# yuxiaoxiangyong/Multilateral-Temporal-view-Pyramid-Transformer-for-Video-Inpainting-Detection

Measured on AMD Instinct MI355X. Metric: clips/sec fwd (B=8,T=5,224x224), higher is better.
Workload: dtype f32; 1 GPU; full Mumpy forward (3 temporal views, pyramid decoder), B=8 clips/GPU, T=5, 224x224, fp32, tubelets (5,4,1); global_batch=8, launch=hipGraph replay, fork/join over HIP streams (independent branches co-scheduled), parallelism=batch-sharded x1, one metric all-reduce

## Files before the change

### include/mumpy_hip.h

```cpp
#ifndef MUMPY_HIP_H
#define MUMPY_HIP_H

#include <stdint.h>

#ifdef __cplusplus
extern "C" {
#endif

#define MUMPY_ABI_VERSION 2

#define MUMPY_EINVAL   (-1)
#define MUMPY_EALIGN   (-2)
#define MUMPY_ENULL    (-3)
#define MUMPY_ERANGE   (-4)

#define MUMPY_ACT_NONE 0
#define MUMPY_ACT_GELU 1
#define MUMPY_MATH_BF16 0x100
#define MUMPY_MATH_BF16X3 0x200
#define MUMPY_MATH_BF16X2 0x400

int         mumpy_abi_version(void);
const char* mumpy_last_error(void);
int         mumpy_tuning_build(void);
// ... 3 lines not shown
int mumpy_linear_rd_fwd(const float* x, const float* W, const float* bias, const float* residual, float* y, int64_t M, int N, int K,
                        int act, void* stream);
int mumpy_window_attention_bg_fwd(const float* qkv, float* out, const float* bias, const float* mask_tab, const int32_t* mask_id,
                                  int n_mask, int B, int Hs, int W, int C, int shift, float scale, void* stream);

int mumpy_linear_ln_tiles(int64_t M, int N, int K);
int mumpy_linear_lnx_fwd(const float* x, const float* W, const float* bias, const float* residual, float* y, int64_t M, int N, int K,
                         int act, void* workspace, int64_t workspace_bytes, float* stats_out, const float* ln_stats, int ln_gn,
                         const float* ln_colsum, float ln_eps, void* stream);

int mumpy_deform_sample_kv_fwd(const float* x2, const float* pos, const float* Wkv, const float* bkv, float* kv, int B, int Hs2,
                               int W, int C, int nq, void* stream);

int mumpy_deform_out_combine_fwd(const float* o, const float* Wout, const float* bout, const float* x1, float* out, int B, int H,
                                 int W, int C, void* stream);

int mumpy_avgpool2_pad_nhwc_fwd(const float* x, float* out, int B, int H, int W, int C, int Cpad, int nchw_in, void* stream);

int mumpy_copy_rows_fwd(const float* src, int64_t src_stride, float* dst, int64_t dst_stride, int64_t rows, int cols, void* stream);

int mumpy_merge_views_fwd(const float* v1, const float* v2, const float* v3, float* out, int B, int T, int n, int C1, int C2,
                          int C3, int t1, int t2, int t3, void* stream);

int mumpy_trunk_head_fwd(const float* g, const float* f, const float* gcn, const float* freq, float* z, int B, int h, int w, int C,
                         void* stream);

int mumpy_layernorm_fwd(const float* x, const float* gamma, const float* beta, float* y,
                        int64_t rows, int C, float eps, void* stream);

int mumpy_layernorm_bf16_fwd(const float* x, const float* gamma, const float* beta, void* y,
// ... 194 lines not shown
```

### multilateral-temporal-view-pyramid-transformer-for-video-inpainting-detection_amd/csrc/abi.cpp

```cpp
#include <stdarg.h>
#include <stdio.h>
#include "common.h"

namespace mumpy {
static thread_local char g_err[512] = "";
void set_error(const char* fmt, ...) {
    va_list ap;
    va_start(ap, fmt);
    vsnprintf(g_err, sizeof(g_err), fmt, ap);
    va_end(ap);
}
#ifdef MUMPY_TUNING
#include <stdlib.h>
int tune_int(const char* name, int dflt) {
    const char* v = getenv(name);
    return v ? atoi(v) : dflt;
}
const char* tune_str(const char* name) { return getenv(name); }
#endif
}

extern "C" int mumpy_tuning_build(void) {
#ifdef MUMPY_TUNING
    return 1;
#else
    return 0;
#endif
}

extern "C" int mumpy_abi_version(void) { return MUMPY_ABI_VERSION; }
extern "C" const char* mumpy_last_error(void) { return mumpy::g_err; }
```

### multilateral-temporal-view-pyramid-transformer-for-video-inpainting-detection_amd/csrc/cva_fused.hip

```cpp
#include "common.h"
using namespace mumpy;

namespace {

constexpr int BK = 32, LDR = 36;

__device__ __forceinline__ void divmod49(unsigned m, unsigned& q, unsigned& r) {
    q = (unsigned)(((uint64_t)m * 2804876602ull) >> 37);
    r = m - 49u * q;
}

template <int C>
__global__ __launch_bounds__(256, 2) void deform_sample_kv_kernel(const float* __restrict__ x2, const float* __restrict__ pos,
                                                                  const float* __restrict__ Wkv, const float* __restrict__ bkv,
                                                                  float* __restrict__ kv, int Hs2, int W, int nWx, int nW2, int nq,
                                                                  int M, unsigned gn) {
    constexpr int BM = 64, BN = 192, TN = 3, N = 2 * C, K = C, CG = C / 3, NK = K / BK, CPG = CG / BK;
    constexpr int A_LD = BM / 32, B_LD = BN / 32;
    __shared__ __attribute__((aligned(16))) float lds[2][(BM + BN) * LDR];
    const int tid = threadIdx.x, lane = tid & 63, wave = tid >> 6;
    const int c = lane & 31, h = lane >> 5, wm = wave >> 1, wn = wave & 1;
    const unsigned nwg = gridDim.x, orig = blockIdx.x, xcd = orig & 7, q8 = nwg >> 3, r8 = nwg & 7;
    const unsigned wgid = (xcd < r8 ? xcd * (q8 + 1) : r8 * (q8 + 1) + (xcd - r8) * q8) + (orig >> 3);
    const unsigned tm = wgid / gn, tn = wgid - tm * gn;
// ... 5 lines not shown
    int aoff[A_LD][4];
    float aw[A_LD][4];
#pragma unroll
    for (int i = 0; i < A_LD; ++i) {
        int m = m0 + ld_row + 32 * i;
        if (m > M - 1) m = M - 1;
        unsigned b2, p;
        divmod49((unsigned)m, b2, p);
        const unsigned b = b2 / (unsigned)nW2, n = b2 - b * (unsigned)nW2;
        const unsigned wy = n / (unsigned)nWx, wx = n - wy * (unsigned)nWx;
        abase[i] = x2 + (((int64_t)b * Hs2 + wy * WS) * W + wx * WS) * C + 4 * ld_c4;
        apos[i] = pos + ((int64_t)(b2 % (unsigned)nq) * 3 * WT + p) * 2;
    }
    auto set_group = [&](int g) {
#pragma unroll
        for (int i = 0; i < A_LD; ++i) {
            const float gy = apos[i][g * WT * 2], gx = apos[i][g * WT * 2 + 1];
            const float iy = ((gy + 1.0f) * 0.5f) * 6.0f;
            const float ix = ((gx + 1.0f) * 0.5f) * 6.0f;
            const float y0f = floorf(iy), x0f = floorf(ix);
            const int y0 = (int)y0f, x0 = (int)x0f;
            const float wgt[4] = {(x0f + 1.0f - ix) * (y0f + 1.0f - iy), (ix - x0f) * (y0f + 1.0f - iy),
                                  (x0f + 1.0f - ix) * (iy - y0f), (ix - x0f) * (iy - y0f)};
#pragma unroll
            for (int e = 0; e < 4; ++e) {
                const int yy = y0 + (e >> 1), xx = x0 + (e & 1);
                const bool ok = (unsigned)yy < (unsigned)WS && (unsigned)xx < (unsigned)WS;
                aw[i][e] = ok ? wgt[e] : 0.f;
                aoff[i][e] = ok ? (yy * W + xx) * C : 0;
            }
        }
    };
    const float* brow[B_LD];
#pragma unroll
    for (int i = 0; i < B_LD; ++i) {
        int n = n0 + ld_row + 32 * i;
        if (n > N - 1) n = N - 1;
        brow[i] = Wkv + (int64_t)n * K + 4 * ld_c4;
    }
    f32x4 areg[A_LD], breg[B_LD];
    auto gload = [&](int kc) {
        const int k0 = kc * BK;
#pragma unroll
        for (int i = 0; i < A_LD; ++i) {
            const float* s = abase[i] + k0;
            f32x4 r = *reinterpret_cast<const f32x4*>(s + aoff[i][0]) * aw[i][0];
            r += *reinterpret_cast<const f32x4*>(s + aoff[i][1]) * aw[i][1];
            r += *reinterpret_cast<const f32x4*>(s + aoff[i][2]) * aw[i][2];
            r += *reinterpret_cast<const f32x4*>(s + aoff[i][3]) * aw[i][3];
            areg[i] = r;
        }
#pragma unroll
        for (int i = 0; i < B_LD; ++i) breg[i] = *reinterpret_cast<const f32x4*>(brow[i] + k0);
    };
    auto lstore = [&](int buf) {
#pragma unroll
        for (int i = 0; i < A_LD; ++i) *reinterpret_cast<f32x4*>(&lds[buf][(ld_row + 32 * i) * LDR + 4 * ld_c4]) = areg[i];
#pragma unroll
        for (int i = 0; i < B_LD; ++i) *reinterpret_cast<f32x4*>(&lds[buf][(BM + ld_row + 32 * i) * LDR + 4 * ld_c4]) = breg[i];
    };
    f32x16 acc[TN];
#pragma unroll
    for (int j = 0; j < TN; ++j)
#pragma unroll
        for (int r = 0; r < 16; ++r) acc[j][r] = 0.f;
// ... 109 lines not shown
    const unsigned b = bw / (unsigned)nWf, n = bw - b * (unsigned)nWf;
    const int wy = (int)(n / (unsigned)nWx), wx = (int)(n - (n / (unsigned)nWx) * (unsigned)nWx);
    const int64_t img = (int64_t)b * H * W;
    const int64_t win_base = (img + (int64_t)n * WT) * C;
#pragma unroll
    for (int r = 0; r < 16; ++r) {
        const int cc = c0 + wm * 32 + (r & 3) + 8 * (r >> 2) + 4 * h;
        if (cc >= C) continue;
        const int f = cc * WT + (int)pp;
        const int po = f / C, co = f - po * C;
        const int tok = window_token(wy, wx, po, H, W, 0);
        out[win_base + f] = x1[win_base + f] + x1[(img + tok) * C + co] + (acc[r] + bout[cc]);
    }
}

}

extern "C" int mumpy_deform_sample_kv_fwd(const float* x2, const float* pos, const float* Wkv, const float* bkv, float* kv, int B,
                                          int Hs2, int W, int C, int nq, void* stream) {
    MUMPY_REQUIRE(x2 && pos && Wkv && bkv && kv, MUMPY_ENULL, "deform_sample_kv: null pointer");
    MUMPY_REQUIRE(aligned16(x2) && aligned16(Wkv) && aligned16(kv), MUMPY_EALIGN, "deform_sample_kv: pointers must be 16-byte aligned");
    MUMPY_REQUIRE(B > 0 && Hs2 > 0 && W > 0 && Hs2 % WS == 0 && W % WS == 0 && nq > 0, MUMPY_EINVAL,
                  "deform_sample_kv: bad grid (%d,%d) / nq=%d", Hs2, W, nq);
    MUMPY_REQUIRE(C == 96 || C == 192 || C == 384 || C == 768, MUMPY_EINVAL,
                  "deform_sample_kv: C=%d is not one of the encoder widths 96/192/384/768", C);
    const int nWx = W / WS, nW2 = (Hs2 / WS) * nWx;
    const int64_t nwin = (int64_t)B * nW2, M = nwin * WT;
    MUMPY_REQUIRE(M < (1ll << 31) - 64, MUMPY_ERANGE, "deform_sample_kv: too many windows");
    const unsigned gn = (unsigned)((2 * C + 191) / 192);
    const int64_t grid = ((M + 63) / 64) * gn;
    MUMPY_REQUIRE(grid < (1ll << 31), MUMPY_ERANGE, "deform_sample_kv: too many tiles");
#define MUMPY_SKV(C_)                                                                                                     \
    hipLaunchKernelGGL(deform_sample_kv_kernel<C_>, dim3((unsigned)grid), dim3(256), 0, as_stream(stream), x2, pos, Wkv, bkv, \
                       kv, Hs2, W, nWx, nW2, nq, (int)M, gn)
    switch (C) {
        case 96: MUMPY_SKV(96); break;
        case 192: MUMPY_SKV(192); break;
        case 384: MUMPY_SKV(384); break;
        default: MUMPY_SKV(768); break;
    }
#undef MUMPY_SKV
    MUMPY_CHECK_LAUNCH("deform_sample_kv");
    return 0;
}

extern "C" int mumpy_deform_out_combine_fwd(const float* o, const float* Wout, const float* bout, const float* x1, float* out, int B,
                                            int H, int W, int C, void* stream) {
    MUMPY_REQUIRE(o && Wout && bout && x1 && out, MUMPY_ENULL, "deform_out_combine: null pointer");
    MUMPY_REQUIRE(x1 != out, MUMPY_EINVAL, "deform_out_combine: out must not alias x1");
    MUMPY_REQUIRE(aligned16(o) && aligned16(Wout), MUMPY_EALIGN, "deform_out_combine: pointers must be 16-byte aligned");
    MUMPY_REQUIRE(B > 0 && H > 0 && W > 0 && H % WS == 0 && W % WS == 0, MUMPY_EINVAL, "deform_out_combine: bad grid (%d,%d)", H, W);
    MUMPY_REQUIRE(C == 96 || C == 192 || C == 384 || C == 768, MUMPY_EINVAL,
                  "deform_out_combine: C=%d is not one of the encoder widths 96/192/384/768", C);
    const int nWx = W / WS, nWf = (H / WS) * nWx;
    const int64_t MO = (int64_t)B * nWf * WT;
    MUMPY_REQUIRE(MO * 49 < (1ll << 31) && MO < (1ll << 31) - 64, MUMPY_ERANGE, "deform_out_combine: too many windows");
    const unsigned gn = (unsigned)((C + 63) / 64);
    const int64_t grid = ((MO + 63) / 64) * gn;
#define MUMPY_OC(C_)                                                                                                      \
    hipLaunchKernelGGL(deform_out_combine_kernel<C_>, dim3((unsigned)grid), dim3(256), 0, as_stream(stream), o, Wout, bout, x1, \
                       out, H, W, nWx, nWf, (int)MO, gn)
    switch (C) {
        case 96: MUMPY_OC(96); break;
        case 192: MUMPY_OC(192); break;
        case 384: MUMPY_OC(384); break;
        default: MUMPY_OC(768); break;
    }
#undef MUMPY_OC
    MUMPY_CHECK_LAUNCH("deform_out_combine");
    return 0;
}
```

### multilateral-temporal-view-pyramid-transformer-for-video-inpainting-detection_amd/csrc/deform.hip

```cpp
#include <stdlib.h>
#include "common.h"
using namespace mumpy;

namespace {

template <int Cg>
__global__ __launch_bounds__(256) void deform_offsets_kernel(const float* __restrict__ q, const float* __restrict__ dw_w,
                                                             const float* __restrict__ dw_b,
                                                             const float* __restrict__ ln_g,
                                                             const float* __restrict__ ln_b,
                                                             const float* __restrict__ pw_w, float* __restrict__ pos,
                                                             int H, int W, int C, int nWx, int nWf) {
    constexpr int CP = Cg + 4;
    __shared__ __attribute__((aligned(16))) float sm[WT * Cg + WT * CP + 25 * Cg + 4 * Cg];
    float* tile = sm;
    float* conv = sm + WT * Cg;
    float* wsm = conv + WT * CP;
    float* par = wsm + 25 * Cg;
    const int bw = blockIdx.x, g = blockIdx.y;
    const int b = bw / nWf, n = bw - b * nWf;
    const int wy = n / nWx, wx = n - wy * nWx;
    const int tid = threadIdx.x;
    const int64_t L = (int64_t)H * W;
    const float* qb = q + (int64_t)b * L * C + g * Cg;
// ... 73 lines not shown
        for (int ch = qd; ch < Cg; ch += 4) {
            const float a = gelu_erf((cv[ch] - mean) * rstd * par[ch] + par[Cg + ch]);
            oy = fmaf(a, par[2 * Cg + ch], oy);
            ox = fmaf(a, par[3 * Cg + ch], ox);
        }
        oy += __shfl_xor(oy, 1);
        oy += __shfl_xor(oy, 2);
        ox += __shfl_xor(ox, 1);
        ox += __shfl_xor(ox, 2);
        if (qd == 0) {
            const int py = p / WS, px = p - py * WS;
            const float ry = ((0.5f + (float)py) / 7.0f) * 2.0f - 1.0f;
            const float rx = ((0.5f + (float)px) / 7.0f) * 2.0f - 1.0f;
            const float rng = 1.0f / 7.0f;
            float* o = pos + (((int64_t)bw * 3 + g) * WT + p) * 2;
            o[0] = tanhf(oy) * rng * 2.0f + ry;
            o[1] = tanhf(ox) * rng * 2.0f + rx;
        }
    }
}

template <int C>
__global__ __launch_bounds__(256) void deform_sample_kernel(const float* __restrict__ x2, const float* __restrict__ pos,
                                                            float* __restrict__ out, int Hs2, int W, int nWx, int nW2,
                                                            int nq) {
    constexpr int C4N = C / 4, CG = C / 3;
    const int b2 = blockIdx.x;
    const int b = b2 / nW2, n = b2 - b * nW2;
    const int wy = n / nWx, wx = n - wy * nWx;
    const float* base = x2 + ((int64_t)b * Hs2 * W + (int64_t)wy * WS * W + wx * WS) * C;
// ... 98 lines not shown
        reinterpret_cast<f32x4*>(o)[i] = reinterpret_cast<const f32x4*>(a)[i] + reinterpret_cast<const f32x4*>(b)[i];
}

}

extern "C" int mumpy_deform_offsets_fwd(const float* q, const float* dw_w, const float* dw_b, const float* ln_g,
                                        const float* ln_b, const float* pw_w, float* pos, int B, int H, int W, int C,
                                        void* stream) {
    MUMPY_REQUIRE(q && dw_w && dw_b && ln_g && ln_b && pw_w && pos, MUMPY_ENULL, "deform_offsets: null pointer");
    MUMPY_REQUIRE(aligned16(q) && aligned16(dw_w), MUMPY_EALIGN, "deform_offsets: q and the depthwise weights must be 16-byte aligned");
    MUMPY_REQUIRE(B > 0 && H % WS == 0 && W % WS == 0 && H > 0 && W > 0, MUMPY_EINVAL, "deform_offsets: bad grid (%d,%d)", H, W);
    const int Cg = C / 3;
    MUMPY_REQUIRE(C % 3 == 0 && (Cg == 32 || Cg == 64 || Cg == 128 || Cg == 256), MUMPY_EINVAL,
                  "deform_offsets: group width C/3=%d must be 32, 64, 128 or 256", Cg);
    const int nWx = W / WS, nWf = (H / WS) * nWx;
#define MUMPY_OFFS(CG)                                                                                              \
    hipLaunchKernelGGL(deform_offsets_kernel<CG>, dim3(B * nWf, 3), dim3(256), 0, as_stream(stream), q, dw_w, dw_b, ln_g, \
                       ln_b, pw_w, pos, H, W, C, nWx, nWf)
    switch (Cg) {
        case 32: MUMPY_OFFS(32); break;
        case 64: MUMPY_OFFS(64); break;
        case 128: MUMPY_OFFS(128); break;
        default: MUMPY_OFFS(256); break;
    }
#undef MUMPY_OFFS
    MUMPY_CHECK_LAUNCH("deform_offsets");
    return 0;
}

extern "C" int mumpy_deform_sample_fwd(const float* x2, const float* pos, float* out, int B, int Hs2, int W, int C,
                                       int nq, void* stream) {
    MUMPY_REQUIRE(x2 && pos && out, MUMPY_ENULL, "deform_sample: null pointer");
    MUMPY_REQUIRE(aligned16(x2) && aligned16(out), MUMPY_EALIGN, "deform_sample: pointers must be 16-byte aligned");
// ... 51 lines not shown
```

### multilateral-temporal-view-pyramid-transformer-for-video-inpainting-detection_amd/csrc/window_attention.hip

```cpp
#include <stdlib.h>
#include <type_traits>
#include "common.h"
using namespace mumpy;

namespace {

struct SelfArgs {
    const float* qkv;
    float* out;
    const float* bias;
    const float* mask_tab;
    const int32_t* mask_id;
    int B, Hs, W, C, nH, shift, nWx, nW, n_mask, groups, stagger;
    int dbg;
    float scale;
    int64_t units;
};

struct CrossArgs {
    const float* q;
    const float* kv;
    const float* padmask;
    float* out;
    int B, H, W, C, nH, r, nWx, nWf, B1w;
// ... 464 lines not shown
#pragma unroll
        for (int it = 0; it < 2; ++it) {
            f32x16 s[2];
#pragma unroll
            for (int jt = 0; jt < 2; ++jt)
#pragma unroll
                for (int r = 0; r < 16; ++r) s[jt][r] = 0.f;
            qk_product(s, kf, qf[it]);
            bias_softmax<false>(s, [&](int jt, int g) {
                f32x4 bv = {0.f, 0.f, 0.f, 0.f};
                if (jt == 1 && g == 2 && h) bv.x = -1e30f;
                return bv;
            }, nullptr, 32 * it + c, h, a.scale);
            pv_product(o[it], s, vf);
        }
    }
    float* obase = a.out + b1 * WT * a.C + head * HD;
    store_o(o[0], 0, [&](int i) { return obase + (int64_t)i * a.C; }, c, h);
    store_o(o[1], 1, [&](int i) { return obase + (int64_t)i * a.C; }, c, h);
}

struct BwdArgs {
    const float* qkv; const float* dout; const float* bias; const float* mask_tab; const int32_t* mask_id;
    float* dqkv; float* stats; float* dbias_part;
    int B, Hs, W, C, nH, shift, nWx, nW, n_mask, groups;
    float scale;
};

__device__ __forceinline__ void load_frag16(f32x4 (&f)[4], const char* base, uint32_t off) {
#pragma unroll
// ... 549 lines not shown
extern "C" int mumpy_deform_attention_fwd(const float* q, const float* kv, const float* padmask, float* out, int B,
                                          int H, int W, int C, int r, float scale, void* stream) {
    MUMPY_REQUIRE(q && kv && padmask && out, MUMPY_ENULL, "deform_attention: null pointer");
    MUMPY_REQUIRE(aligned16(q) && aligned16(kv) && aligned16(padmask) && aligned16(out), MUMPY_EALIGN,
                  "deform_attention: pointers must be 16-byte aligned");
    MUMPY_REQUIRE(B > 0 && H > 0 && W > 0 && H % WS == 0 && W % WS == 0 && r >= 1, MUMPY_EINVAL,
                  "deform_attention: bad grid (%d,%d) or ratio %d", H, W, r);
    MUMPY_REQUIRE(C > 0 && C % HD == 0, MUMPY_EINVAL, "deform_attention: C=%d not a multiple of 32", C);
    CrossArgs a;
    a.q = q; a.kv = kv; a.padmask = padmask; a.out = out;
    a.B = B; a.H = H; a.W = W; a.C = C; a.nH = C / HD; a.r = r;
    a.nWx = W / WS; a.nWf = (H / WS) * (W / WS); a.B1w = B * a.nWf; a.scale = scale;
    a.units = (int64_t)a.B1w * a.nH;
    const int64_t grid = (a.units + 3) / 4;
    MUMPY_REQUIRE(grid < (1ll << 31), MUMPY_ERANGE, "deform_attention: too many windows");
    hipLaunchKernelGGL(win_attn_cross_kernel, dim3((unsigned)grid), dim3(256), 0, as_stream(stream), a);
    MUMPY_CHECK_LAUNCH("deform_attention");
    return 0;
}

static int64_t wa_bwd_groups(int B, int nW, int nH) {
    const int64_t quads = ((int64_t)B * nW + 3) / 4;
    static const int target = tune_int("MUMPY_WA_BWD_BLOCKS", 256);
    int64_t groups = (target + nH - 1) / nH;
    return groups > quads ? quads : groups;
}

extern "C" int64_t mumpy_window_attention_bwd_workspace_bytes(int B, int Hs, int W, int C) {
    if (B <= 0 || Hs <= 0 || W <= 0 || C <= 0 || Hs % WS || W % WS || C % HD) return 0;
    const int nW = (Hs / WS) * (W / WS), nH = C / HD;
    const int64_t stats = (int64_t)B * nW * nH * 192;
// ... 99 lines not shown
```

### multilateral-temporal-view-pyramid-transformer-for-video-inpainting-detection_amd/mumpy_hip/lib.py

```python
import ctypes
import os
import subprocess

_HERE = os.path.dirname(os.path.abspath(__file__))
_PKG = os.path.dirname(_HERE)
_LIB = None

c_f = ctypes.c_void_p
c_i = ctypes.c_int
c_l = ctypes.c_int64
c_fl = ctypes.c_float
c_d = ctypes.c_double

SIGNATURES = {
    "mumpy_layernorm_fwd": [c_f, c_f, c_f, c_f, c_l, c_i, c_fl, c_f],
    "mumpy_layernorm_bf16_fwd": [c_f, c_f, c_f, c_f, c_l, c_i, c_fl, c_f],
    "mumpy_linear_fwd": [c_f, c_f, c_f, c_f, c_f, c_l, c_i, c_i, c_i, c_f],
    "mumpy_linear_bf16s_fwd": [c_f, c_f, c_f, c_f, c_f, c_l, c_i, c_i, c_i, c_i, c_f],
    "mumpy_window_attention_bf16_fwd": [c_f, c_f, c_f, c_f, c_f, c_i, c_i, c_i, c_i, c_i, c_i, c_fl, c_f],
    "mumpy_window_attention_bf16mm_fwd": [c_f, c_f, c_f, c_f, c_f, c_i, c_i, c_i, c_i, c_i, c_i, c_fl, c_f],
    "mumpy_linear_ws_fwd": [c_f, c_f, c_f, c_f, c_f, c_l, c_i, c_i, c_i, c_f, c_l, c_f],
    "mumpy_linear_wsz_fwd": [c_f, c_f, c_f, c_f, c_f, c_l, c_i, c_i, c_i, c_f, c_l, c_f],
    "mumpy_linear_rd_fwd": [c_f, c_f, c_f, c_f, c_f, c_l, c_i, c_i, c_i, c_f],
    "mumpy_window_attention_bg_fwd": [c_f, c_f, c_f, c_f, c_f, c_i, c_i, c_i, c_i, c_i, c_i, c_fl, c_f],
# ... 8 lines not shown
    "mumpy_gn_apply_resample_nhwc_fwd": [c_f, c_f, c_i, c_f, c_f, c_i, c_fl, c_i, c_i, c_i, c_i, c_i, c_f, c_f, c_f, c_i, c_i,
                                         c_i, c_i, c_i, c_i, c_f],
    "mumpy_conv2d_nhwc_fwd": [c_f, c_f, c_f, c_f, c_f, c_i, c_i, c_i, c_i, c_i, c_i, c_i, c_i, c_f, c_l, c_f],
    "mumpy_conv2d_workspace_bytes": [c_i, c_i, c_i, c_i, c_i, c_i, c_i],
    "mumpy_avgpool2_pad_nhwc_fwd": [c_f, c_f, c_i, c_i, c_i, c_i, c_i, c_i, c_f],
    "mumpy_copy_rows_fwd": [c_f, c_l, c_f, c_l, c_l, c_i, c_f],
    "mumpy_merge_views_fwd": [c_f, c_f, c_f, c_f, c_i, c_i, c_i, c_i, c_i, c_i, c_i, c_i, c_i, c_f],
    "mumpy_trunk_head_fwd": [c_f, c_f, c_f, c_f, c_f, c_i, c_i, c_i, c_i, c_f],
    "mumpy_final_conv_fwd": [c_f, c_f, c_f, c_f, c_f, c_i, c_i, c_i, c_i, c_fl, c_f],
    "mumpy_window_attention_fwd": [c_f, c_f, c_f, c_f, c_f, c_i, c_i, c_i, c_i, c_i, c_i, c_fl, c_f],
    "mumpy_deform_offsets_fwd": [c_f, c_f, c_f, c_f, c_f, c_f, c_f, c_i, c_i, c_i, c_i, c_f],
    "mumpy_deform_sample_fwd": [c_f, c_f, c_f, c_i, c_i, c_i, c_i, c_i, c_f],
    "mumpy_deform_attention_fwd": [c_f, c_f, c_f, c_f, c_i, c_i, c_i, c_i, c_i, c_fl, c_f],
    "mumpy_deform_sample_kv_fwd": [c_f, c_f, c_f, c_f, c_f, c_i, c_i, c_i, c_i, c_i, c_f],
    "mumpy_deform_out_combine_fwd": [c_f, c_f, c_f, c_f, c_f, c_i, c_i, c_i, c_i, c_f],
    "mumpy_deform_combine_fwd": [c_f, c_f, c_f, c_i, c_i, c_i, c_i, c_f],
    "mumpy_faf_fwd": [c_f, c_f, c_f, c_f, c_f, c_i, c_i, c_i, c_i, c_i, c_i, c_f],
    "mumpy_patch_embed_fwd": [c_f, c_f, c_f, c_f, c_f, c_f, c_i, c_i, c_i, c_i, c_i, c_i, c_fl, c_f],
    "mumpy_patch_merge_ln_fwd": [c_f, c_f, c_f, c_f, c_i, c_i, c_i, c_i, c_fl, c_f],
    "mumpy_temporal_attention_fwd": [c_f, c_f, c_l, c_i, c_i, c_i, c_fl, c_f],
    "mumpy_attention_probs_fwd": [c_f, c_f, c_f, c_l, c_i, c_i, c_i, c_i, c_l, c_l, c_l, c_l, c_l, c_fl, c_f],
    "mumpy_temporal_attention_q_fwd": [c_f, c_f, c_l, c_i, c_i, c_i, c_i, c_fl, c_f],
    "mumpy_sigmoid_threshold_fwd": [c_f, c_f, c_l, c_fl, c_f],
    "mumpy_add_fwd": [c_f, c_f, c_f, c_l, c_f],
    "mumpy_normalize_u8_fwd": [c_f, c_f, c_l, c_i, c_i, ctypes.POINTER(ctypes.c_float), ctypes.POINTER(ctypes.c_float), c_f],
    "mumpy_resize_nearest_table": [c_i, c_i, ctypes.POINTER(ctypes.c_int32)],
    "mumpy_resize_normalize_u8_fwd": [c_f, c_f, c_f, c_f, c_l, c_i, c_i, c_i, c_i, ctypes.POINTER(ctypes.c_float), ctypes.POINTER(ctypes.c_float), c_f],
    "mumpy_mask_loss_workspace_bytes": [c_i, c_l],
    "mumpy_mask_loss_fwd_bwd": [c_f, c_f, c_f, c_f, c_f, c_l, c_i, c_l, c_fl, c_fl, c_f],
    "mumpy_layernorm_bwd_workspace_bytes": [c_l, c_i],
# ... 83 lines not shown
```

Before: 374.9 clips/s.

## Add small-grid variants for cross-view attention kernels when tile counts underfill GPU

Adds a heuristic that detects when the cross-view attention stage (offsets, sample-KV GEMM, out-combine GEMM, deform attention) would launch too few workgroups. For those cases it selects new kernel variants: smaller tiles with multi-stage register prefetch for the GEMMs, a per-row grid split for the offsets kernel, and a split-r attention kernel that reduces partial outputs through shared memory. The aim is more parallelism on deep pyramid levels with few windows, at the cost of extra partial-sum traffic and more code paths. The bilinear corner math is factored into helpers with explicit FMA ordering so both paths give consistent numerics.

```diff
diff --git a/include/mumpy_hip.h b/include/mumpy_hip.h
--- a/include/mumpy_hip.h
+++ b/include/mumpy_hip.h
@@ -41,6 +41,12 @@
 
 int mumpy_deform_out_combine_fwd(const float* o, const float* Wout, const float* bout, const float* x1, float* out, int B, int H,
                                  int W, int C, void* stream);
+
+#define MUMPY_CVA_OFFSETS     0
+#define MUMPY_CVA_SAMPLE_KV   1
+#define MUMPY_CVA_OUT_COMBINE 2
+#define MUMPY_CVA_ATTENTION   3
+int mumpy_cva_small_grid(int kernel, int64_t windows, int C, int r);
 
 int mumpy_avgpool2_pad_nhwc_fwd(const float* x, float* out, int B, int H, int W, int C, int Cpad, int nchw_in, void* stream);
 
diff --git a/multilateral-temporal-view-pyramid-transformer-for-video-inpainting-detection_amd/csrc/abi.cpp b/multilateral-temporal-view-pyramid-transformer-for-video-inpainting-detection_amd/csrc/abi.cpp
--- a/multilateral-temporal-view-pyramid-transformer-for-video-inpainting-detection_amd/csrc/abi.cpp
+++ b/multilateral-temporal-view-pyramid-transformer-for-video-inpainting-detection_amd/csrc/abi.cpp
@@ -30,3 +30,15 @@
 
 extern "C" int mumpy_abi_version(void) { return MUMPY_ABI_VERSION; }
 extern "C" const char* mumpy_last_error(void) { return mumpy::g_err; }
+
+extern "C" int mumpy_cva_small_grid(int kernel, int64_t windows, int C, int r) {
+    if (windows <= 0 || C <= 0) return MUMPY_EINVAL;
+    const int64_t rows = windows * 49;
+    switch (kernel) {
+        case MUMPY_CVA_OFFSETS: return windows * 3 < 512;
+        case MUMPY_CVA_SAMPLE_KV: return 2 * C > 192 && ((rows + 63) / 64) * ((2 * C + 191) / 192) < 512;
+        case MUMPY_CVA_OUT_COMBINE: return ((rows + 63) / 64) * ((C + 63) / 64) < 512;
+        case MUMPY_CVA_ATTENTION: return r > 1 && r <= 8 && (windows * (C / 32) + 3) / 4 < 128;
+        default: return MUMPY_EINVAL;
+    }
+}
diff --git a/multilateral-temporal-view-pyramid-transformer-for-video-inpainting-detection_amd/csrc/cva_fused.hip b/multilateral-temporal-view-pyramid-transformer-for-video-inpainting-detection_amd/csrc/cva_fused.hip
--- a/multilateral-temporal-view-pyramid-transformer-for-video-inpainting-detection_amd/csrc/cva_fused.hip
+++ b/multilateral-temporal-view-pyramid-transformer-for-video-inpainting-detection_amd/csrc/cva_fused.hip
@@ -4,10 +4,42 @@
 namespace {
 
 constexpr int BK = 32, LDR = 36;
+#ifndef MUMPY_CVA_SETS
+#define MUMPY_CVA_SETS 2
+#endif
+constexpr int CVA_SETS = MUMPY_CVA_SETS;
 
 __device__ __forceinline__ void divmod49(unsigned m, unsigned& q, unsigned& r) {
     q = (unsigned)(((uint64_t)m * 2804876602ull) >> 37);
     r = m - 49u * q;
+}
+
+__device__ __forceinline__ void corner_weights(float gy, float gx, int W, int C, int (&off)[4], float (&w)[4]) {
+#pragma clang fp contract(off)
+    const float iy = ((gy + 1.0f) * 0.5f) * 6.0f;
+    const float ix = ((gx + 1.0f) * 0.5f) * 6.0f;
+    const float y0f = floorf(iy), x0f = floorf(ix);
+    const int y0 = (int)y0f, x0 = (int)x0f;
+    const float wgt[4] = {(x0f + 1.0f - ix) * (y0f + 1.0f - iy), (ix - x0f) * (y0f + 1.0f - iy),
+                          (x0f + 1.0f - ix) * (iy - y0f), (ix - x0f) * (iy - y0f)};
+#pragma unroll
+    for (int e = 0; e < 4; ++e) {
+        const int yy = y0 + (e >> 1), xx = x0 + (e & 1);
+        const bool ok = (unsigned)yy < (unsigned)WS && (unsigned)xx < (unsigned)WS;
+        w[e] = ok ? wgt[e] : 0.f;
+        off[e] = ok ? (yy * W + xx) * C : 0;
+    }
+}
+__device__ __forceinline__ f32x4 corner_sum(f32x4 c0, f32x4 c1, f32x4 c2, f32x4 c3, const float (&w)[4]) {
+    f32x4 r;
+    {
+#pragma clang fp contract(off)
+        r = c0 * w[0];
+    }
+    r = __builtin_elementwise_fma(c1, f32x4{w[1], w[1], w[1], w[1]}, r);
+    r = __builtin_elementwise_fma(c2, f32x4{w[2], w[2], w[2], w[2]}, r);
+    r = __builtin_elementwise_fma(c3, f32x4{w[3], w[3], w[3], w[3]}, r);
+    return r;
 }
 
 template <int C>
@@ -43,22 +75,7 @@
     }
     auto set_group = [&](int g) {
 #pragma unroll
-        for (int i = 0; i < A_LD; ++i) {
-            const float gy = apos[i][g * WT * 2], gx = apos[i][g * WT * 2 + 1];
-            const float iy = ((gy + 1.0f) * 0.5f) * 6.0f;
-            const float ix = ((gx + 1.0f) * 0.5f) * 6.0f;
-            const float y0f = floorf(iy), x0f = floorf(ix);
-            const int y0 = (int)y0f, x0 = (int)x0f;
-            const float wgt[4] = {(x0f + 1.0f - ix) * (y0f + 1.0f - iy), (ix - x0f) * (y0f + 1.0f - iy),
-                                  (x0f + 1.0f - ix) * (iy - y0f), (ix - x0f) * (iy - y0f)};
-#pragma unroll
-            for (int e = 0; e < 4; ++e) {
-                const int yy = y0 + (e >> 1), xx = x0 + (e & 1);
-                const bool ok = (unsigned)yy < (unsigned)WS && (unsigned)xx < (unsigned)WS;
-                aw[i][e] = ok ? wgt[e] : 0.f;
-                aoff[i][e] = ok ? (yy * W + xx) * C : 0;
-            }
-        }
+        for (int i = 0; i < A_LD; ++i) corner_weights(apos[i][g * WT * 2], apos[i][g * WT * 2 + 1], W, C, aoff[i], aw[i]);
     };
     const float* brow[B_LD];
 #pragma unroll
@@ -73,11 +90,8 @@
 #pragma unroll
         for (int i = 0; i < A_LD; ++i) {
             const float* s = abase[i] + k0;
-            f32x4 r = *reinterpret_cast<const f32x4*>(s + aoff[i][0]) * aw[i][0];
-            r += *reinterpret_cast<const f32x4*>(s + aoff[i][1]) * aw[i][1];
-            r += *reinterpret_cast<const f32x4*>(s + aoff[i][2]) * aw[i][2];
-            r += *reinterpret_cast<const f32x4*>(s + aoff[i][3]) * aw[i][3];
-            areg[i] = r;
+            areg[i] = corner_sum(*reinterpret_cast<const f32x4*>(s + aoff[i][0]), *reinterpret_cast<const f32x4*>(s + aoff[i][1]),
+                                 *reinterpret_cast<const f32x4*>(s + aoff[i][2]), *reinterpret_cast<const f32x4*>(s + aoff[i][3]), aw[i]);
         }
 #pragma unroll
         for (int i = 0; i < B_LD; ++i) breg[i] = *reinterpret_cast<const f32x4*>(brow[i] + k0);
@@ -217,6 +231,200 @@
     }
 }
 
+template <int C, int S>
+__global__ __launch_bounds__(256, 2) void deform_sample_kv_small_kernel(const float* __restrict__ x2, const float* __restrict__ pos,
+                                                                        const float* __restrict__ Wkv, const float* __restrict__ bkv,
+                                                                        float* __restrict__ kv, int Hs2, int W, int nWx, int nW2,
+                                                                        int nq, int M, unsigned gn) {
+    constexpr int BM = 64, BN = 64, N = 2 * C, K = C, CG = C / 3, NK = K / BK, CPG = CG / BK;
+    constexpr int A_LD = BM / 32, B_LD = BN / 32;
+    __shared__ __attribute__((aligned(16))) float lds[2][(BM + BN) * LDR];
+    const int tid = threadIdx.x, lane = tid & 63, wave = tid >> 6;
+    const int c = lane & 31, h = lane >> 5, wm = wave >> 1, wn = wave & 1;
+    const unsigned nwg = gridDim.x, orig = blockIdx.x, xcd = orig & 7, q8 = nwg >> 3, r8 = nwg & 7;
+    const unsigned wgid = (xcd < r8 ? xcd * (q8 + 1) : r8 * (q8 + 1) + (xcd - r8) * q8) + (orig >> 3);
+    const unsigned tm = wgid / gn, tn = wgid - tm * gn;
+    const int m0 = (int)tm * BM, n0 = (int)tn * BN;
+    const int ld_row = tid >> 3, ld_c4 = tid & 7;
+
+    const float* abase[A_LD];
+    float gpos[A_LD][3][2];
+    int aoff[A_LD][4];
+    float aw[A_LD][4];
+#pragma unroll
+    for (int i = 0; i < A_LD; ++i) {
+        int m = m0 + ld_row + 32 * i;
+        if (m > M - 1) m = M - 1;
+        unsigned b2, p;
+        divmod49((unsigned)m, b2, p);
+        const unsigned b = b2 / (unsigned)nW2, n = b2 - b * (unsigned)nW2;
+        const unsigned wy = n / (unsigned)nWx, wx = n - wy * (unsigned)nWx;
+        abase[i] = x2 + (((int64_t)b * Hs2 + wy * WS) * W + wx * WS) * C + 4 * ld_c4;
+        const float* ap = pos + ((int64_t)(b2 % (unsigned)nq) * 3 * WT + p) * 2;
+#pragma unroll
+        for (int g = 0; g < 3; ++g) { gpos[i][g][0] = ap[g * WT * 2]; gpos[i][g][1] = ap[g * WT * 2 + 1]; }
+    }
+    auto set_group = [&](int g) {
+#pragma unroll
+        for (int i = 0; i < A_LD; ++i) {
+            const float gy = g == 0 ? gpos[i][0][0] : g == 1 ? gpos[i][1][0] : gpos[i][2][0];
+            const float gx = g == 0 ? gpos[i][0][1] : g == 1 ? gpos[i][1][1] : gpos[i][2][1];
+            corner_weights(gy, gx, W, C, aoff[i], aw[i]);
+        }
+    };
+    const float* brow[B_LD];
+#pragma unroll
+    for (int i = 0; i < B_LD; ++i) brow[i] = Wkv + (int64_t)(n0 + ld_row + 32 * i) * K + 4 * ld_c4;
+
+    f32x4 ra[S][A_LD][4], rb[S][B_LD];
+    float rw[S][A_LD][4];
+    auto gload = [&](int kc, int s) {
+        if (kc % CPG == 0) set_group(kc / CPG);
+        const int k0 = kc * BK;
+#pragma unroll
+        for (int i = 0; i < A_LD; ++i)
+#pragma unroll
+            for (int e = 0; e < 4; ++e) {
+                ra[s][i][e] = *reinterpret_cast<const f32x4*>(abase[i] + k0 + aoff[i][e]);
+                rw[s][i][e] = aw[i][e];
+            }
+#pragma unroll
+        for (int i = 0; i < B_LD; ++i) rb[s][i] = *reinterpret_cast<const f32x4*>(brow[i] + k0);
+    };
+    auto lstore = [&](int buf, int s) {
+#pragma unroll
+        for (int i = 0; i < A_LD; ++i) {
+            const f32x4 r = corner_sum(ra[s][i][0], ra[s][i][1], ra[s][i][2], ra[s][i][3], rw[s][i]);
+            *reinterpret_cast<f32x4*>(&lds[buf][(ld_row + 32 * i) * LDR + 4 * ld_c4]) = r;
+        }
+#pragma unroll
+        for (int i = 0; i < B_LD; ++i) *reinterpret_cast<f32x4*>(&lds[buf][(BM + ld_row + 32 * i) * LDR + 4 * ld_c4]) = rb[s][i];
+    };
+    f32x16 acc;
+#pragma unroll
+    for (int r = 0; r < 16; ++r) acc[r] = 0.f;
+    auto compute = [&](int buf) {
+        const float* a_f = &lds[buf][(wm * 32 + c) * LDR + 16 * h];
+        const float* b_f = &lds[buf][(BM + wn * 32 + c) * LDR + 16 * h];
+#pragma unroll
+        for (int q = 0; q < 4; ++q) {
+            const f32x4 fa = *reinterpret_cast<const f32x4*>(a_f + 4 * q), fb = *reinterpret_cast<const f32x4*>(b_f + 4 * q);
+#pragma unroll
+            for (int e = 0; e < 4; ++e) acc = __builtin_amdgcn_mfma_f32_32x32x2f32(fa[e], fb[e], acc, 0, 0, 0);
+        }
+    };
+#pragma unroll
+    for (int s = 0; s < S; ++s)
+        if (s < NK) gload(s, s);
+    lstore(0, 0);
+    __syncthreads();
+    for (int kc0 = 0; kc0 < NK; kc0 += S) {
+#pragma unroll
+        for (int u = 0; u < S; ++u) {
+            const int kc = kc0 + u;
+            if (kc < NK) {
+                if (kc + S < NK) gload(kc + S, u);
+                compute(kc & 1);
+                if (kc + 1 < NK) lstore((kc + 1) & 1, (u + 1) % S);
+                __syncthreads();
+            }
+        }
+    }
+    const int n = n0 + wn * 32 + c;
+    const float bv = bkv[n];
+#pragma unroll
+    for (int r = 0; r < 16; ++r) {
+        const int m = m0 + wm * 32 + (r & 3) + 8 * (r >> 2) + 4 * h;
+        if (m < M) kv[(int64_t)m * N + n] = acc[r] + bv;
+    }
+}
+
+template <int C, int S>
+__global__ __launch_bounds__(128, 4) void deform_out_combine_small_kernel(const float* __restrict__ o, const float* __restrict__ Wout,
+                                                                         const float* __restrict__ bout, const float* __restrict__ x1,
+                                                                         float* __restrict__ out, int H, int W, int nWx, int nWf,
+                                                                         int MO, unsigned gn) {
+    constexpr int BM = 32, BN = 64, K = C, NK = K / BK;
+    constexpr int A_LD = BM / 16, B_LD = BN / 16;
+    __shared__ __attribute__((aligned(16))) float lds[2][(BM + BN) * LDR];
+    const int tid = threadIdx.x, lane = tid & 63, wn = tid >> 6;
+    const int c = lane & 31, h = lane >> 5;
+    const unsigned nwg = gridDim.x, orig = blockIdx.x, xcd = orig & 7, q8 = nwg >> 3, r8 = nwg & 7;
+    const unsigned wgid = (xcd < r8 ? xcd * (q8 + 1) : r8 * (q8 + 1) + (xcd - r8) * q8) + (orig >> 3);
+    const unsigned tn = wgid / gn, tm = wgid - tn * gn;
+    const int c0 = (int)tm * BM, m0 = (int)tn * BN;
+    const int ld_row = tid >> 3, ld_c4 = tid & 7;
+    const float* arow[A_LD];
+    const float* brow[B_LD];
+#pragma unroll
+    for (int i = 0; i < A_LD; ++i) arow[i] = Wout + (int64_t)(c0 + ld_row + 16 * i) * K + 4 * ld_c4;
+#pragma unroll
+    for (int i = 0; i < B_LD; ++i) {
+        int m = m0 + ld_row + 16 * i;
+        if (m > MO - 1) m = MO - 1;
+        brow[i] = o + (int64_t)m * K + 4 * ld_c4;
+    }
+    f32x4 ra[S][A_LD], rb[S][B_LD];
+    auto gload = [&](int kc, int s) {
+#pragma unroll
+        for (int i = 0; i < A_LD; ++i) ra[s][i] = *reinterpret_cast<const f32x4*>(arow[i] + kc * BK);
+#pragma unroll
+        for (int i = 0; i < B_LD; ++i) rb[s][i] = *reinterpret_cast<const f32x4*>(brow[i] + kc * BK);
+    };
+    auto lstore = [&](int buf, int s) {
+#pragma unroll
+        for (int i = 0; i < A_LD; ++i) *reinterpret_cast<f32x4*>(&lds[buf][(ld_row + 16 * i) * LDR + 4 * ld_c4]) = ra[s][i];
+#pragma unroll
+        for (int i = 0; i < B_LD; ++i) *reinterpret_cast<f32x4*>(&lds[buf][(BM + ld_row + 16 * i) * LDR + 4 * ld_c4]) = rb[s][i];
+    };
+    f32x16 acc;
+#pragma unroll
+    for (int r = 0; r < 16; ++r) acc[r] = 0.f;
+    auto compute = [&](int buf) {
+        const float* a_f = &lds[buf][c * LDR + 16 * h];
+        const float* b_f = &lds[buf][(BM + wn * 32 + c) * LDR + 16 * h];
+#pragma unroll
+        for (int q = 0; q < 4; ++q) {
+            const f32x4 fa = *reinterpret_cast<const f32x4*>(a_f + 4 * q), fb = *reinterpret_cast<const f32x4*>(b_f + 4 * q);
+#pragma unroll
+            for (int e = 0; e < 4; ++e) acc = __builtin_amdgcn_mfma_f32_32x32x2f32(fa[e], fb[e], acc, 0, 0, 0);
+        }
+    };
+#pragma unroll
+    for (int s = 0; s < S; ++s)
+        if (s < NK) gload(s, s);
+    lstore(0, 0);
+    __syncthreads();
+    for (int kc0 = 0; kc0 < NK; kc0 += S) {
+#pragma unroll
+        for (int u = 0; u < S; ++u) {
+            const int kc = kc0 + u;
+            if (kc < NK) {
+                if (kc + S < NK) gload(kc + S, u);
+                compute(kc & 1);
+                if (kc + 1 < NK) lstore((kc + 1) & 1, (u + 1) % S);
+                __syncthreads();
+            }
+        }
+    }
+    const int m = m0 + wn * 32 + c;
+    if (m >= MO) return;
+    unsigned bw, pp;
+    divmod49((unsigned)m, bw, pp);
+    const unsigned b = bw / (unsigned)nWf, n = bw - b * (unsigned)nWf;
+    const int wy = (int)(n / (unsigned)nWx), wx = (int)(n - (n / (unsigned)nWx) * (unsigned)nWx);
+    const int64_t img = (int64_t)b * H * W;
+    const int64_t win_base = (img + (int64_t)n * WT) * C;
+#pragma unroll
+    for (int r = 0; r < 16; ++r) {
+        const int cc = c0 + (r & 3) + 8 * (r >> 2) + 4 * h;
+        const int f = cc * WT + (int)pp;
+        const int po = f / C, co = f - po * C;
+        const int tok = window_token(wy, wx, po, H, W, 0);
+        out[win_base + f] = x1[win_base + f] + x1[(img + tok) * C + co] + (acc[r] + bout[cc]);
+    }
+}
+
 }
 
 extern "C" int mumpy_deform_sample_kv_fwd(const float* x2, const float* pos, const float* Wkv, const float* bkv, float* kv, int B,
@@ -230,12 +438,18 @@
     const int nWx = W / WS, nW2 = (Hs2 / WS) * nWx;
     const int64_t nwin = (int64_t)B * nW2, M = nwin * WT;
     MUMPY_REQUIRE(M < (1ll << 31) - 64, MUMPY_ERANGE, "deform_sample_kv: too many windows");
-    const unsigned gn = (unsigned)((2 * C + 191) / 192);
+    const int force = tune_int("MUMPY_CVA_FORCE", 0);
+    const bool small = force ? force == 2 : mumpy_cva_small_grid(MUMPY_CVA_SAMPLE_KV, nwin, C, 1) != 0;
+    const unsigned gn = small ? (unsigned)(2 * C / 64) : (unsigned)((2 * C + 191) / 192);
     const int64_t grid = ((M + 63) / 64) * gn;
     MUMPY_REQUIRE(grid < (1ll << 31), MUMPY_ERANGE, "deform_sample_kv: too many tiles");
 #define MUMPY_SKV(C_)                                                                                                     \
-    hipLaunchKernelGGL(deform_sample_kv_kernel<C_>, dim3((unsigned)grid), dim3(256), 0, as_stream(stream), x2, pos, Wkv, bkv, \
-                       kv, Hs2, W, nWx, nW2, nq, (int)M, gn)
+    if (small)                                                                                                            \
+        hipLaunchKernelGGL((deform_sample_kv_small_kernel<C_, CVA_SETS>), dim3((unsigned)grid), dim3(256), 0, as_stream(stream), x2, \
+                           pos, Wkv, bkv, kv, Hs2, W, nWx, nW2, nq, (int)M, gn);                                          \
+    else                                                                                                                  \
+        hipLaunchKernelGGL(deform_sample_kv_kernel<C_>, dim3((unsigned)grid), dim3(256), 0, as_stream(stream), x2, pos, Wkv, bkv, \
+                           kv, Hs2, W, nWx, nW2, nq, (int)M, gn)
     switch (C) {
         case 96: MUMPY_SKV(96); break;
         case 192: MUMPY_SKV(192); break;
@@ -258,11 +472,17 @@
     const int nWx = W / WS, nWf = (H / WS) * nWx;
     const int64_t MO = (int64_t)B * nWf * WT;
     MUMPY_REQUIRE(MO * 49 < (1ll << 31) && MO < (1ll << 31) - 64, MUMPY_ERANGE, "deform_out_combine: too many windows");
-    const unsigned gn = (unsigned)((C + 63) / 64);
+    const int force = tune_int("MUMPY_CVA_FORCE", 0);
+    const bool small = force ? force == 2 : mumpy_cva_small_grid(MUMPY_CVA_OUT_COMBINE, (int64_t)B * nWf, C, 1) != 0;
+    const unsigned gn = small ? (unsigned)(C / 32) : (unsigned)((C + 63) / 64);
     const int64_t grid = ((MO + 63) / 64) * gn;
 #define MUMPY_OC(C_)                                                                                                      \
-    hipLaunchKernelGGL(deform_out_combine_kernel<C_>, dim3((unsigned)grid), dim3(256), 0, as_stream(stream), o, Wout, bout, x1, \
-                       out, H, W, nWx, nWf, (int)MO, gn)
+    if (small)                                                                                                            \
+        hipLaunchKernelGGL((deform_out_combine_small_kernel<C_, CVA_SETS>), dim3((unsigned)grid), dim3(128), 0, as_stream(stream), o, \
+                           Wout, bout, x1, out, H, W, nWx, nWf, (int)MO, gn);                                             \
+    else                                                                                                                  \
+        hipLaunchKernelGGL(deform_out_combine_kernel<C_>, dim3((unsigned)grid), dim3(256), 0, as_stream(stream), o, Wout, bout, x1, \
+                           out, H, W, nWx, nWf, (int)MO, gn)
     switch (C) {
         case 96: MUMPY_OC(96); break;
         case 192: MUMPY_OC(192); break;
diff --git a/multilateral-temporal-view-pyramid-transformer-for-video-inpainting-detection_amd/csrc/deform.hip b/multilateral-temporal-view-pyramid-transformer-for-video-inpainting-detection_amd/csrc/deform.hip
--- a/multilateral-temporal-view-pyramid-transformer-for-video-inpainting-detection_amd/csrc/deform.hip
+++ b/multilateral-temporal-view-pyramid-transformer-for-video-inpainting-detection_amd/csrc/deform.hip
@@ -111,6 +111,118 @@
             const float rx = ((0.5f + (float)px) / 7.0f) * 2.0f - 1.0f;
             const float rng = 1.0f / 7.0f;
             float* o = pos + (((int64_t)bw * 3 + g) * WT + p) * 2;
+            o[0] = tanhf(oy) * rng * 2.0f + ry;
+            o[1] = tanhf(ox) * rng * 2.0f + rx;
+        }
+    }
+}
+
+template <int Cg>
+__global__ __launch_bounds__(256) void deform_offsets_rows_kernel(const float* __restrict__ q, const float* __restrict__ dw_w,
+                                                                  const float* __restrict__ dw_b,
+                                                                  const float* __restrict__ ln_g,
+                                                                  const float* __restrict__ ln_b,
+                                                                  const float* __restrict__ pw_w, float* __restrict__ pos,
+                                                                  int H, int W, int C, int nWx, int nWf) {
+    constexpr int CP = Cg + 4, TR = 5;
+    __shared__ __attribute__((aligned(16))) float sm[TR * WS * Cg + WS * CP + 25 * Cg + 4 * Cg];
+    float* tile = sm;
+    float* conv = sm + TR * WS * Cg;
+    float* wsm = conv + WS * CP;
+    float* par = wsm + 25 * Cg;
+    const int bw = blockIdx.x, g = blockIdx.y, py = blockIdx.z;
+    const int b = bw / nWf, n = bw - b * nWf;
+    const int wy = n / nWx, wx = n - wy * nWx;
+    const int tid = threadIdx.x;
+    const int64_t L = (int64_t)H * W;
+    const float* qb = q + (int64_t)b * L * C + g * Cg;
+    const int cg4 = Cg >> 2;
+    {
+        constexpr int NT = TR * WS * (Cg / 4), PT = (NT + 255) / 256;
+        f32x4 v[PT];
+#pragma unroll
+        for (int u = 0; u < PT; ++u) {
+            const int idx = tid + 256 * u;
+            const int lp = idx / cg4, c4 = idx - lp * cg4;
+            const int yy = py - 2 + lp / WS;
+            if (idx < NT && (unsigned)yy < (unsigned)WS)
+                v[u] = *reinterpret_cast<const f32x4*>(qb + (int64_t)window_token(wy, wx, yy * WS + lp % WS, H, W, 0) * C + 4 * c4);
+        }
+#pragma unroll
+        for (int u = 0; u < PT; ++u) {
+            const int idx = tid + 256 * u;
+            const int lp = idx / cg4, c4 = idx - lp * cg4;
+            const int yy = py - 2 + lp / WS;
+            if (idx < NT && (unsigned)yy < (unsigned)WS) *reinterpret_cast<f32x4*>(tile + lp * Cg + 4 * c4) = v[u];
+        }
+        constexpr int NW = 25 * Cg / 4, PW = (NW + 255) / 256;
+        f32x4 t[PW];
+#pragma unroll
+        for (int u = 0; u < PW; ++u) { const int idx = tid + 256 * u; if (idx < NW) t[u] = reinterpret_cast<const f32x4*>(dw_w)[idx]; }
+#pragma unroll
+        for (int u = 0; u < PW; ++u) { const int idx = tid + 256 * u; if (idx < NW) reinterpret_cast<f32x4*>(wsm)[idx] = t[u]; }
+    }
+    for (int idx = tid; idx < Cg; idx += 256) {
+        par[idx] = ln_g[idx];
+        par[Cg + idx] = ln_b[idx];
+        par[2 * Cg + idx] = pw_w[idx];
+        par[3 * Cg + idx] = pw_w[Cg + idx];
+    }
+    const int cc = tid % Cg;
+    const float breg = dw_b[cc];
+    __syncthreads();
+    float wreg[25];
+#pragma unroll
+    for (int i = 0; i < 25; ++i) wreg[i] = wsm[cc * 25 + i];
+    for (int px = tid / Cg; px < WS; px += 256 / Cg) {
+        float acc = breg;
+#pragma unroll
+        for (int dy = 0; dy < 5; ++dy) {
+            const bool vy = (unsigned)(py + dy - 2) < (unsigned)WS;
+            const int lr = vy ? dy : 2;
+#pragma unroll
+            for (int dx = 0; dx < 5; ++dx) {
+                const int xx = px + dx - 2;
+                const bool ok = vy && (unsigned)xx < (unsigned)WS;
+                const int xc = ok ? xx : px;
+                const float t = tile[((ok ? lr : 2) * WS + xc) * Cg + cc];
+                acc = fmaf(ok ? t : 0.f, wreg[dy * 5 + dx], acc);
+            }
+        }
+        conv[px * CP + cc] = acc;
+    }
+    __syncthreads();
+    const int px = tid >> 2, qd = tid & 3;
+    if (px < WS) {
+        const float* cv = conv + px * CP;
+        float s = 0.f;
+#pragma unroll 8
+        for (int ch = qd; ch < Cg; ch += 4) s += cv[ch];
+        s += __shfl_xor(s, 1);
+        s += __shfl_xor(s, 2);
+        const float mean = s / (float)Cg;
+        float qq = 0.f;
+#pragma unroll 8
+        for (int ch = qd; ch < Cg; ch += 4) { const float d = cv[ch] - mean; qq = fmaf(d, d, qq); }
+        qq += __shfl_xor(qq, 1);
+        qq += __shfl_xor(qq, 2);
+        const float rstd = rsqrtf(qq / (float)Cg + 1e-5f);
+        float oy = 0.f, ox = 0.f;
+#pragma unroll 4
+        for (int ch = qd; ch < Cg; ch += 4) {
+            const float a = gelu_erf((cv[ch] - mean) * rstd * par[ch] + par[Cg + ch]);
+            oy = fmaf(a, par[2 * Cg + ch], oy);
+            ox = fmaf(a, par[3 * Cg + ch], ox);
+        }
+        oy += __shfl_xor(oy, 1);
+        oy += __shfl_xor(oy, 2);
+        ox += __shfl_xor(ox, 1);
+        ox += __shfl_xor(ox, 2);
+        if (qd == 0) {
+            const float ry = ((0.5f + (float)py) / 7.0f) * 2.0f - 1.0f;
+            const float rx = ((0.5f + (float)px) / 7.0f) * 2.0f - 1.0f;
+            const float rng = 1.0f / 7.0f;
+            float* o = pos + (((int64_t)bw * 3 + g) * WT + py * WS + px) * 2;
             o[0] = tanhf(oy) * rng * 2.0f + ry;
             o[1] = tanhf(ox) * rng * 2.0f + rx;
         }
@@ -239,9 +351,15 @@
     MUMPY_REQUIRE(C % 3 == 0 && (Cg == 32 || Cg == 64 || Cg == 128 || Cg == 256), MUMPY_EINVAL,
                   "deform_offsets: group width C/3=%d must be 32, 64, 128 or 256", Cg);
     const int nWx = W / WS, nWf = (H / WS) * nWx;
+    const int force = tune_int("MUMPY_CVA_FORCE", 0);
+    const bool rows = force ? force == 2 : mumpy_cva_small_grid(MUMPY_CVA_OFFSETS, (int64_t)B * nWf, C, 1) != 0;
 #define MUMPY_OFFS(CG)                                                                                              \
-    hipLaunchKernelGGL(deform_offsets_kernel<CG>, dim3(B * nWf, 3), dim3(256), 0, as_stream(stream), q, dw_w, dw_b, ln_g, \
-                       ln_b, pw_w, pos, H, W, C, nWx, nWf)
+    if (rows)                                                                                                       \
+        hipLaunchKernelGGL(deform_offsets_rows_kernel<CG>, dim3(B * nWf, 3, WS), dim3(256), 0, as_stream(stream), q, dw_w, dw_b, \
+                           ln_g, ln_b, pw_w, pos, H, W, C, nWx, nWf);                                               \
+    else                                                                                                            \
+        hipLaunchKernelGGL(deform_offsets_kernel<CG>, dim3(B * nWf, 3), dim3(256), 0, as_stream(stream), q, dw_w, dw_b, ln_g, \
+                           ln_b, pw_w, pos, H, W, C, nWx, nWf)
     switch (Cg) {
         case 32: MUMPY_OFFS(32); break;
         case 64: MUMPY_OFFS(64); break;
diff --git a/multilateral-temporal-view-pyramid-transformer-for-video-inpainting-detection_amd/csrc/window_attention.hip b/multilateral-temporal-view-pyramid-transformer-for-video-inpainting-detection_amd/csrc/window_attention.hip
--- a/multilateral-temporal-view-pyramid-transformer-for-video-inpainting-detection_amd/csrc/window_attention.hip
+++ b/multilateral-temporal-view-pyramid-transformer-for-video-inpainting-detection_amd/csrc/window_attention.hip
@@ -502,6 +502,78 @@
             }, nullptr, 32 * it + c, h, a.scale);
             pv_product(o[it], s, vf);
         }
+    }
+    float* obase = a.out + b1 * WT * a.C + head * HD;
+    store_o(o[0], 0, [&](int i) { return obase + (int64_t)i * a.C; }, c, h);
+    store_o(o[1], 1, [&](int i) { return obase + (int64_t)i * a.C; }, c, h);
+}
+
+__global__ __launch_bounds__(512) void win_attn_cross_split_kernel(CrossArgs a) {
+    extern __shared__ __attribute__((aligned(16))) float cross_sm[];
+    const int lane = threadIdx.x & 63, t = threadIdx.x >> 6;
+    const int c = lane & 31, h = lane >> 5;
+    const int64_t u = blockIdx.x;
+    const int head = (int)(u % a.nH);
+    const int64_t b1 = u / a.nH;
+    int* tt = reinterpret_cast<int*>(cross_sm) + 64 * t;
+    float* part = cross_sm + 64 * a.r;
+    const int64_t L = (int64_t)a.H * a.W;
+    f32x16 o[2];
+#pragma unroll
+    for (int it = 0; it < 2; ++it)
+#pragma unroll
+        for (int r = 0; r < 16; ++r) o[it][r] = 0.f;
+    {
+        const int64_t b2 = b1 * a.r + t;
+        const int qw = (int)(b2 % a.B1w);
+        const int qb = qw / a.nWf, qn = qw - qb * a.nWf;
+        const int wy = qn / a.nWx, wx = qn - wy * a.nWx;
+        tt[lane] = (lane < WT) ? window_token(wy, wx, lane, a.H, a.W, 0) : 0;
+        __builtin_amdgcn_wave_barrier();
+        const float* qbase = a.q + ((int64_t)qb * L) * a.C + head * HD;
+        const float* kbase = a.kv + b2 * WT * 2 * a.C + head * HD;
+        f32x4 qf[2][4], kf[2][4];
+#pragma unroll
+        for (int tl = 0; tl < 2; ++tl) {
+            const int p = 32 * tl + c;
+            const bool valid = p < WT;
+            load_frag(qf[tl], qbase + (int64_t)tt[p & 63] * a.C + 16 * h, valid);
+            load_frag(kf[tl], kbase + (int64_t)(valid ? p : 0) * 2 * a.C + 16 * h, valid);
+        }
+        float vf[2][16];
+        const float* vbase = kbase + a.C;
+        load_v(vf, [&](int j) { return vbase + (int64_t)j * 2 * a.C; }, c, h);
+#pragma unroll
+        for (int it = 0; it < 2; ++it) {
+            f32x16 s[2];
+#pragma unroll
+            for (int jt = 0; jt < 2; ++jt)
+#pragma unroll
+                for (int r = 0; r < 16; ++r) s[jt][r] = 0.f;
+            qk_product(s, kf, qf[it]);
+            bias_softmax<false>(s, [&](int jt, int g) {
+                f32x4 bv = {0.f, 0.f, 0.f, 0.f};
+                if (jt == 1 && g == 2 && h) bv.x = -1e30f;
+                return bv;
+            }, nullptr, 32 * it + c, h, a.scale);
+            pv_product(o[it], s, vf);
+        }
+    }
+    if (t > 0) {
+        float* pw = part + (int64_t)(t - 1) * 32 * 64 + lane;
+#pragma unroll
+        for (int it = 0; it < 2; ++it)
+#pragma unroll
+            for (int r = 0; r < 16; ++r) pw[(16 * it + r) * 64] = o[it][r];
+    }
+    __syncthreads();
+    if (t > 0) return;
+    for (int k = 1; k < a.r; ++k) {
+        const float* pr = part + (int64_t)(k - 1) * 32 * 64 + lane;
+#pragma unroll
+        for (int it = 0; it < 2; ++it)
+#pragma unroll
+            for (int r = 0; r < 16; ++r) o[it][r] += pr[(16 * it + r) * 64];
     }
     float* obase = a.out + b1 * WT * a.C + head * HD;
     store_o(o[0], 0, [&](int i) { return obase + (int64_t)i * a.C; }, c, h);
@@ -1081,7 +1153,14 @@
     a.units = (int64_t)a.B1w * a.nH;
     const int64_t grid = (a.units + 3) / 4;
     MUMPY_REQUIRE(grid < (1ll << 31), MUMPY_ERANGE, "deform_attention: too many windows");
-    hipLaunchKernelGGL(win_attn_cross_kernel, dim3((unsigned)grid), dim3(256), 0, as_stream(stream), a);
+    const int force = tune_int("MUMPY_CVA_FORCE", 0);
+    const bool split = r > 1 && r <= 8 && a.units < (1ll << 31) &&
+                       (force ? force == 2 : mumpy_cva_small_grid(MUMPY_CVA_ATTENTION, a.B1w, C, r) != 0);
+    if (split)
+        hipLaunchKernelGGL(win_attn_cross_split_kernel, dim3((unsigned)a.units), dim3(64 * r),
+                           (size_t)(64 * r + (r - 1) * 32 * 64) * sizeof(float), as_stream(stream), a);
+    else
+        hipLaunchKernelGGL(win_attn_cross_kernel, dim3((unsigned)grid), dim3(256), 0, as_stream(stream), a);
     MUMPY_CHECK_LAUNCH("deform_attention");
     return 0;
 }
diff --git a/multilateral-temporal-view-pyramid-transformer-for-video-inpainting-detection_amd/mumpy_hip/lib.py b/multilateral-temporal-view-pyramid-transformer-for-video-inpainting-detection_amd/mumpy_hip/lib.py
--- a/multilateral-temporal-view-pyramid-transformer-for-video-inpainting-detection_amd/mumpy_hip/lib.py
+++ b/multilateral-temporal-view-pyramid-transformer-for-video-inpainting-detection_amd/mumpy_hip/lib.py
@@ -46,6 +46,7 @@
     "mumpy_deform_attention_fwd": [c_f, c_f, c_f, c_f, c_i, c_i, c_i, c_i, c_i, c_fl, c_f],
     "mumpy_deform_sample_kv_fwd": [c_f, c_f, c_f, c_f, c_f, c_i, c_i, c_i, c_i, c_i, c_f],
     "mumpy_deform_out_combine_fwd": [c_f, c_f, c_f, c_f, c_f, c_i, c_i, c_i, c_i, c_f],
+    "mumpy_cva_small_grid": [c_i, c_l, c_i, c_i],
     "mumpy_deform_combine_fwd": [c_f, c_f, c_f, c_i, c_i, c_i, c_i, c_f],
     "mumpy_faf_fwd": [c_f, c_f, c_f, c_f, c_f, c_i, c_i, c_i, c_i, c_i, c_i, c_f],
     "mumpy_patch_embed_fwd": [c_f, c_f, c_f, c_f, c_f, c_f, c_i, c_i, c_i, c_i, c_i, c_i, c_fl, c_f],
```

Result: no change. 377.9 clips/s, median of 6 (+0.8%).
